# SYNCC-IN/hyperscanning-signal-analysis

Hardware: AMD Instinct MI355X
Metric: MVAR+ffDTF windows/sec, 2x32-ch dyad p=8, 256 freqs (higher is better)
Workload: dtype f64; 1 GPU; C2: 1 dyad(s)/GPU, 2x32 ch @500 Hz, 10 min, 2 s windows 50% overlap (599 windows per dyad), MVAR p=8, 256 freqs 0.5-128 Hz; dyads_per_gpu=1, k1=hop blocks summed once, shared by the overlapping windows (hop 500), k2=block Levinson-Whittle recursion, one workgroup per window, one launch, normalisation=inside K3 (rows of window w by workgroups of window w+lag), parallelism=dyad-sharded x1, gather=none

## Files before the change

### hyperscanning_signal_analysis_amd/csrc/capi.hip

```cpp
#include "../../include/hypermvar.h"
#include "hmv_kernels.h"

#include <atomic>
#include <cmath>
#include <cstdio>
#include <cstdlib>
#include <cstring>

namespace {
thread_local char g_err[256] = "";

int fail(int code, const char* msg) {
  snprintf(g_err, sizeof(g_err), "%s", msg);
  return code;
}
int pad_of(int m) { return (m < 1 || m > HMV_MAX_CHANNELS) ? -1 : ((m + 15) / 16) * 16; }
inline hipStream_t S(void* s) { return reinterpret_cast<hipStream_t>(s); }
inline size_t align256(size_t b) { return (b + 255) & ~size_t(255); }

constexpr int N_TUNE = 6;
struct TuneRange { long long lo, hi; };
constexpr TuneRange kTuneRange[N_TUNE] = {{0, 0}, {0, 1 << 20}, {0, 3}, {0, 2}, {0, 3}, {0, 140000}};
long long env_knob(const char* name, int key) {
  const char* e = getenv(name);
  if (!e || !*e) return 0;
  char* end = nullptr;
  const long long v = strtoll(e, &end, 10);
  if (end == e || *end != 0 || v < kTuneRange[key].lo || v > kTuneRange[key].hi) {
    fprintf(stderr, "hypermvar: ignoring %s=%s (not an integer in %lld..%lld)\n", name, e, kTuneRange[key].lo,
            kTuneRange[key].hi);
    return 0;
  }
  return v;
}
std::atomic<long long> g_tune[N_TUNE] = {{0}, {env_knob("HYPERMVAR_NORM_LAG", 1)}, {env_knob("HYPERMVAR_LAG_GROUP", 2)},
                                         {env_knob("HYPERMVAR_K3_FORM", 3)}, {env_knob("HYPERMVAR_YW_FORM", 4)},
                                         {env_knob("HYPERMVAR_K3_LDS_PAD", 5)}};
}

namespace hmv {
long long tuning(int key) { return (key >= 1 && key < N_TUNE) ? g_tune[key].load(std::memory_order_relaxed) : -1; }
}

#ifdef HMV_STAMP
static unsigned long long* g_tf_stamps = nullptr;
extern "C" void hmv_debug_set_tf_stamps(void* p) { g_tf_stamps = static_cast<unsigned long long*>(p); }
#endif

extern "C" {

int hmv_version(void) { return HMV_VERSION; }
const char* hmv_last_error(void) { return g_err; }
int hmv_pad(int m) { return pad_of(m); }

int hmv_set_tuning(int key, int64_t value) {
// ... 398 lines not shown
  TfFfWs w;
  size_t o = 0;
  const size_t t = (size_t)mp * mp;
  w.off_arx = o;    o += align256(sizeof(double) * hmv::tf_workspace_doubles(n, mp, p));
  w.off_P = o;      o += align256(sizeof(double) * n * F * t);
  w.off_rowsum = o; o += align256(sizeof(double) * n * F * mp);
  w.off_cnt = o;    o += align256(sizeof(int) * (2 * n + 1 + n * mp));
  w.off_tail = o;
  if (bands) {
    const int64_t lag = norm_lag_items(mp, F);
    o += align256(sizeof(double) * (size_t)(n < lag ? n : lag) * F * t);
  }
  w.total = o;
  return w;
}
int64_t norm_lag_items(int mp, int F) {
  const int64_t slots = (mp == 64 || mp == 48) ? 1024 : (mp == 32 ? 2048 : 5120);
  int64_t lag = (6 * slots + F - 1) / (F < 1 ? 1 : F);
  if (const int64_t t = hmv::tuning(HMV_TUNE_NORM_LAG)) lag = t;
  return lag < 8 ? 8 : lag;
}
}

int64_t hmv_tf_ffdtf_workspace_bytes(int64_t n_items, int m, int p, int F) {
  const int mp = pad_of(m);
  if (mp < 0 || n_items < 0 || p < 1 || F < 1) return -1;
  return (int64_t)tf_ff_layout(n_items, mp, p, F).total;
}

namespace {
int tf_ffdtf_impl(const char* who, const double* ar, int64_t n_items, int m, int p, const double* tw, int F, double* ffdtf,
                  double* band_out, const int32_t* bin_lo, const int32_t* bin_hi, int n_bands, double* den, double* H,
                  int32_t* info, double pivot_tau, void* workspace, int64_t workspace_bytes, int64_t flags,
                  void* ev_k3_start, void* ev_k3_stop, void* stream) {
  auto failw = [&](int code, const char* msg) {
    char buf[200];
    snprintf(buf, sizeof(buf), "%s: %s", who, msg);
    return fail(code, buf);
  };
  const int mp = pad_of(m);
  const bool bands = (band_out != nullptr);
  if (mp < 0) return failw(-1, "channel count must be in 1..64");
  if (p < 1) return failw(-2, "model order must be >= 1");
  if (n_items == 0) return 0;
  if (!ar || !tw || (!ffdtf && !bands) || !den || !info || !workspace || n_items < 0 || F < 1)
    return failw(-4, "null pointer / empty grid");
  if (!(pivot_tau > 0.0) || pivot_tau > 1.0) return failw(-6, "pivot_tau must be in (0, 1]");
  if (bands) {
    if (!bin_lo || !bin_hi || n_bands < 1) return failw(-4, "band bins missing");
    if (F % 32 != 0 || F > hmv::tf_band_max_F(mp) || (flags & HMV_FLAG_UNFUSED_NORM))
      return failw(-10, "in-kernel band sums need F % 32 == 0, F within the row worker's LDS block and the fused normalisation");
  }
  const TfFfWs w = tf_ff_layout(n_items, mp, p, F, bands);
  if ((int64_t)w.total > workspace_bytes) return failw(-7, "workspace too small");
  char* base = static_cast<char*>(workspace);
  const size_t t = (size_t)mp * mp;
  hmv::TfArgs a{};
  a.ar = ar; a.arx = reinterpret_cast<double*>(base + w.off_arx); a.tw = tw;
  a.P = reinterpret_cast<double*>(base + w.off_P); a.rowsum = reinterpret_cast<double*>(base + w.off_rowsum);
  a.H = H;
  a.info = info; a.n_items = n_items; a.F = F; a.p = p; a.m = m; a.tau = pivot_tau;
  const bool fused = bands || (!(flags & HMV_FLAG_UNFUSED_NORM) && (F % 16 == 0) && (reinterpret_cast<uintptr_t>(ffdtf) % 16 == 0));
  const int64_t lag = norm_lag_items(mp, F);
  const int64_t n_fused = fused ? n_items : 0;
  if (n_fused > 0) {
    a.ff = bands ? nullptr : ffdtf; a.den = den; a.fuse_items = n_fused; a.lag = (int)lag;
    if (bands) {
      a.bands = band_out; a.band_lo = reinterpret_cast<const int*>(bin_lo); a.band_hi = reinterpret_cast<const int*>(bin_hi);
      a.nb = n_bands;
    }
    a.wcount = reinterpret_cast<int*>(base + w.off_cnt);
    a.ready = a.wcount + n_items;
    a.missed = a.ready + n_items;
  }
#ifdef HMV_STAMP
  a.stamps = g_tf_stamps;
#endif
  hipStream_t st = S(stream);
  int rc = hmv::launch_tf_inv(a, mp, st, reinterpret_cast<hipEvent_t>(ev_k3_start), reinterpret_cast<hipEvent_t>(ev_k3_stop));
  if (rc) return rc;
  if (n_fused < n_items) {
    const int64_t n_tail = n_items - n_fused;
    double* tail = bands ? reinterpret_cast<double*>(base + w.off_tail) : ffdtf + (size_t)n_fused * m * m * F;
    rc = hmv_ffdtf_norm_f64(a.P + (size_t)n_fused * F * t, a.rowsum + (size_t)n_fused * F * mp, den + (size_t)n_fused * mp,
                            tail, n_tail, F, m, 1, stream);
    if (!rc && bands)
      rc = hmv::launch_band_sums(tail, reinterpret_cast<const int*>(bin_lo), reinterpret_cast<const int*>(bin_hi),
                                 band_out + (size_t)n_fused * m * m * n_bands, n_tail * (long long)m * m, F, n_bands, st);
  }
  return rc;
}
}

int64_t hmv_tf_ffdtf_bands_workspace_bytes(int64_t n_items, int m, int p, int F) {
  const int mp = pad_of(m);
  if (mp < 0 || n_items < 0 || p < 1 || F < 1) return -1;
  return (int64_t)tf_ff_layout(n_items, mp, p, F, true).total;
}

int hmv_tf_ffdtf_f64(const double* ar, int64_t n_items, int m, int p, const double* tw, int F, double* ffdtf,
                     double* den, double* H, int32_t* info, double pivot_tau, void* workspace, int64_t workspace_bytes,
                     int64_t flags, void* ev_k3_start, void* ev_k3_stop, void* stream) {
  return tf_ffdtf_impl("hmv_tf_ffdtf_f64", ar, n_items, m, p, tw, F, ffdtf, nullptr, nullptr, nullptr, 0, den, H, info,
                       pivot_tau, workspace, workspace_bytes, flags, ev_k3_start, ev_k3_stop, stream);
}

int hmv_tf_ffdtf_bands_f64(const double* ar, int64_t n_items, int m, int p, const double* tw, int F, double* band_out,
                           const int32_t* bin_lo, const int32_t* bin_hi, int n_bands, double* den, int32_t* info,
                           double pivot_tau, void* workspace, int64_t workspace_bytes, int64_t flags, void* ev_k3_start,
                           void* ev_k3_stop, void* stream) {
  if (!band_out) return fail(-4, "hmv_tf_ffdtf_bands_f64: null pointer / empty grid");
  return tf_ffdtf_impl("hmv_tf_ffdtf_bands_f64", ar, n_items, m, p, tw, F, nullptr, band_out, bin_lo, bin_hi, n_bands, den,
// ... 243 lines not shown
    } else {
      rc = hmv_lagcov_f64(a.x, a.rec_stride, a.ld, a.item_rec + i0, a.item_start + i0, c, a.m, a.n, a.p, R, st0);
    }
    if (rc) break;
    if (automatic) {
      hmv::YwArgs ya{};
      ya.R = R; ya.n_items = c; ya.m = a.m; ya.p = a.p; ya.ws = ws; ya.ar = ar_c; ya.V = V_c; ya.info = a.info_yw + i0;
      ya.tiled = -1;
      hmv::YwAutoArgs sel{};
      sel.n = a.n; sel.crit_c = crit_factor(a.crit, a.n); sel.order_out = a.order_out + i0;
      sel.crit_out = a.crit_out ? a.crit_out + (size_t)i0 * a.p : nullptr;
      rc = hmv::launch_yw_auto(ya, sel, mp, st0);
      if (rc) break;
    }
    const bool ldl = (a.flags & (HMV_FLAG_YW_TILED | HMV_FLAG_YW_ONE_LAUNCH)) || hmv::tuning(HMV_TUNE_YW_FORM) == 1;
    const bool tiled = (a.flags & HMV_FLAG_YW_TILED) || (ldl && !(a.flags & HMV_FLAG_YW_ONE_LAUNCH) && mp == 64 && c >= 128);
    const int64_t yw_flags = (a.flags & ~(int64_t)(HMV_FLAG_YW_TILED | HMV_FLAG_YW_ONE_LAUNCH)) |
                             (ldl ? (tiled ? HMV_FLAG_YW_TILED : HMV_FLAG_YW_ONE_LAUNCH) : 0);
    const int64_t c0 = (split && tiled && c >= 16) ? (c + 1) / 2 : c, c1 = c - c0;
    if (c1 > 0 && !automatic) {
      int hrc = (int)hipEventRecord(fj->fork, st0);
      if (!hrc) hrc = (int)hipStreamWaitEvent(st1, fj->fork, 0);
      if (hrc) { rc = hrc; break; }
      rc = hmv_yw_solve_f64(R + (size_t)c0 * (a.p + 1) * t, c1, a.m, a.p, ws + (size_t)c0 * ws_item,
                            ar_c + (size_t)c0 * t * a.p, V_c + (size_t)c0 * t, nullptr, a.info_yw + i0 + c0, yw_flags, st1);
      hrc = (int)hipEventRecord(fj->join, st1);
      if (!hrc) hrc = (int)hipStreamWaitEvent(st0, fj->join, 0);
      if (hrc) {
        (void)hipStreamSynchronize(st1);
        if (!rc) rc = hrc;
      }
      if (rc) break;
    }
    if (!automatic) rc = hmv_yw_solve_f64(R, c0, a.m, a.p, ws, ar_c, V_c, nullptr, a.info_yw + i0, yw_flags, st0);
    if (rc) break;
    const bool last = (ci == n_chunks - 1);
    double* Hc = a.S_out ? reinterpret_cast<double*>(base + w.off_H) : nullptr;
    double* full_c = (a.measure == MEAS_FFDTF) ? nullptr
                     : bands ? reinterpret_cast<double*>(base + w.off_full) : a.ffdtf + (size_t)i0 * a.m * a.m * a.F;
    if (a.measure == MEAS_GPDC) {
      rc = hmv::launch_gpdc_sliding(ar_c, V_c, tw, full_c, c, a.F, a.m, mp, a.p, st0);
    } else {
      rc = tf_ffdtf_impl(a.who, ar_c, c, a.m, a.p, tw, a.F,
                         k3_bands ? nullptr : (full_c ? full_c : a.ffdtf + (size_t)i0 * a.m * a.m * a.F),
                         k3_bands ? a.band_out + (size_t)i0 * a.m * a.m * a.n_bands : nullptr, a.bin_lo, a.bin_hi,
                         a.n_bands, den, Hc, a.info_tf + (size_t)i0 * a.F, a.pivot_tau, tfws, tfws_bytes, a.flags,
                         last ? a.ev_k3_start : nullptr, last ? a.ev_k3_stop : nullptr, st0);
    }
    if (!rc && a.measure == MEAS_DDTF) {
      hmv::DdtfArgs da{};
      da.ar = ar_c; da.V = V_c; da.info_yw = a.info_yw + i0;
      da.B = reinterpret_cast<double*>(base + w.off_B); da.G = reinterpret_cast<double*>(base + w.off_G);
      da.freqs = a.freqs; da.fs = a.fs; da.ff = full_c; da.out = full_c;
      da.n_items = c; da.F = a.F; da.m = a.m; da.p = a.p;
      rc = hmv::launch_ddtf_sliding(da, mp, st0);
    }
    if (!rc && a.measure != MEAS_FFDTF && bands)
      rc = hmv::launch_band_sums(full_c, reinterpret_cast<const int*>(a.bin_lo), reinterpret_cast<const int*>(a.bin_hi),
                                 a.band_out + (size_t)i0 * a.m * a.m * a.n_bands, c * (long long)a.m * a.m, a.F,
                                 a.n_bands, st0);
    if (!rc && a.S_out) {
      hmv::SpecArgs sa;
      sa.H = Hc; sa.V = V_c; sa.S = nullptr; sa.S_mmf = a.S_out + (size_t)i0 * a.m * a.m * a.F * 2;
      sa.n_items = c; sa.F = a.F; sa.m = a.m; sa.sym = 1;
      rc = hmv::launch_spectra(sa, mp, st0);
    }
  }
  return rc;
}
}

int64_t hmv_sliding_bands_workspace_bytes(int64_t chunk, int m, int p, int F) { return sliding_bytes(chunk, m, p, F, 1); }

int hmv_sliding_ffdtf_f64(const double* x, int64_t rec_stride, int64_t ld, const int64_t* item_rec,
                          const int64_t* item_start, int64_t n_items, int m, int n, int p,
                          const double* freqs, int F, double fs, double* ffdtf, double* ar_out, double* V_out,
                          int32_t* info_yw, int32_t* info_tf, void* workspace, int64_t workspace_bytes,
                          int64_t chunk, double pivot_tau, int64_t flags, int64_t grid_hop, int64_t grid_first,
                          int64_t grid_nwin, int64_t grid_T, void* ev_k3_start, void* ev_k3_stop, void* stream,
                          void* aux_stream) {
// ... 519 lines not shown
```

### hyperscanning_signal_analysis_amd/csrc/hmv_kernels.h

```cpp
#pragma once
#include <hip/hip_runtime.h>
#include <stdint.h>

namespace hmv {

long long tuning(int key);

struct LagcovArgs {
  const double* x;
  long long rec_stride;
  long long ld;
  const long long* item_rec;
  const long long* item_start;
  long long n_items;
  int m, n, p;
  double* R;
  int blocks;
  long long blk_first, blk_T;
};
int launch_lagcov(const LagcovArgs& a, int m_pad, hipStream_t st);
struct LagcombArgs {
  const double* Q;
  const double* x;
  long long ld, first, hop, T;
// ... 34 lines not shown
  const long long* rec_b;
  const long long* item_start;
  long long n_items;
  int m, n, p, split;
  double* R;
  const double* R_base;
  const long long* base_a;
  const long long* base_b;
};
int launch_lagcov_pairs(const LagcovPairsArgs& a, int m_pad, hipStream_t st);
struct LagcovMixArgs {
  const double* Rt;
  const double* W;
  const double* scale;
  long long n_trials, n_win;
  long long it0, n_items;
  int m, m_pad, p;
  double* R;
};
int launch_lagcov_mix(const LagcovMixArgs& a, hipStream_t st);

struct YwArgs {
  const double* R;
  long long n_items;
  int m, p;
  double* ws;
  double* ar;
  double* V;
  double* Vq_logdet;
  int* info;
  int tiled;
  int only_guarded;
  const int* order;
};
struct YwAutoArgs {
  int n;
  double crit_c;
  int* order_out;
  double* crit_out;
};
long long yw_ws_tiles(int p);
int launch_yw(const YwArgs& a, int m_pad, hipStream_t st);
int launch_yw_lwr(const YwArgs& a, int m_pad, hipStream_t st);
int launch_yw_lwr2(const YwArgs& a, int m_pad, hipStream_t st);
int launch_yw_auto(const YwArgs& a, const YwAutoArgs& s, int m_pad, hipStream_t st);
int launch_yw_guarded(const YwArgs& a, int m_pad, hipStream_t st);

struct TfArgs {
  const double* ar;
  const double* arx;
  const double* tw;
  const double* Zin;
  double* detph;
  double* P;
  double* rowsum;
  double* H;
  double* A;
  int* info;
  long long n_items;
  int F, p, m;
  double tau;
  double* ff;
  double* den;
  int* wcount;
  int* ready;
  int* missed;
  long long fuse_items;
  int lag;
  double* bands;
  const int* band_lo;
  const int* band_hi;
  int nb;
  unsigned long long* stamps;
};
int launch_twiddles(const double* freqs, int F, double fs, int p, double* tw, hipStream_t st);
int launch_tf_inv(const TfArgs& a, int m_pad, hipStream_t st, hipEvent_t ev_start = nullptr, hipEvent_t ev_stop = nullptr);
int launch_cinv(const TfArgs& a, int m_pad, hipStream_t st);
long long tf_workspace_doubles(long long n_items, int m_pad, int p);
int tf_band_max_F(int m_pad);

struct NormArgs {
  const double* P;
  const double* rowsum;
  double* den;
  double* out;
  long long n_items;
  int F, m, m_pad;
  int normalise;
};
int launch_ffdtf_norm(const NormArgs& a, hipStream_t st);

int launch_trial_mean(const double* in, double* out, long long n, int trials, hipStream_t st);
int launch_ddtf(const double* ff, const double* kappa, double* out, long long n, hipStream_t st);
int launch_band_sums(const double* in, const int* lo, const int* hi, double* out, long long rows, int F, int nb,
                     hipStream_t st);

int launch_transpose_c128(const double* in, double* out, long long n_items, int F, int m, int m_pad, hipStream_t st);

struct SpecArgs {
  const double* H;
  const double* V;
  double* S;
  double* S_mmf;
  long long n_items;
  int F, m;
  int sym;
};
int launch_spectra(const SpecArgs& a, int m_pad, hipStream_t st);

// ... 107 lines not shown
```

### hyperscanning_signal_analysis_amd/csrc/tf_inv.hip

```cpp
#include "hmv_common.h"
#include "hmv_kernels.h"

namespace hmv {

#ifndef HMV_K3_WGS
#define HMV_K3_WGS 4
#endif

#ifndef HMV_ROW_LOADS_SC1
#define HMV_ROW_LOADS_SC1 0
#endif

#define HMV_LDS_FENCE()                                     \
  do {                                                      \
    __builtin_amdgcn_fence(__ATOMIC_RELEASE, "wavefront");  \
    __builtin_amdgcn_wave_barrier();                        \
    __builtin_amdgcn_fence(__ATOMIC_ACQUIRE, "wavefront");  \
  } while (0)

#ifdef HMV_STAMP
#define HMV_T(idx)                                                                     \
  do {                                                                                 \
    __builtin_amdgcn_sched_barrier(0);                                                 \
    unsigned long long t_;                                                             \
// ... 794 lines not shown
  {
    const unsigned long long d[8] = {q0 & 0xffffffffull, q0 >> 32, q1 & 0xffffffffull, q1 >> 32,
                                     q2 & 0xffffffffull, q2 >> 32, q3 & 0xffffffffull, q3 >> 32};
    tsum[0] = d[0]; tsum[2] = d[1]; tsum[3] = d[2] + d[3] + d[4]; tsum[1] = d[5] + d[6] + d[7];
    unsigned long long now;
    asm volatile("s_memtime %0\n\ts_waitcnt lgkmcnt(0)" : "=s"(now)::"memory");
    tlast = (now & ~0xffffffffull) | tl32;
    if (tlast > now) tlast -= 0x100000000ull;
    if (a.stamps && lane_id() == 0) {
      unsigned long long* det = a.stamps + ((size_t)a.n_items * a.F * NT + (size_t)(gw * NT + wv)) * 8;
      for (int k = 0; k < 8; ++k) det[k] = d[k];
    }
  }
#else
  K3A_BODY(acc, arx, tw, p, w, tau, ldsbase);
#endif
  double re[NT][4], im[NT][4];
#pragma unroll
  for (int Ig = 0; Ig < 4; ++Ig)
#pragma unroll
    for (int Jl = 0; Jl < 4; ++Jl) {
      re[Ig][Jl] = acc[2 * (4 * Ig + Jl)];
      im[Ig][Jl] = acc[2 * (4 * Ig + Jl) + 1];
    }
  double2* smem = reinterpret_cast<double2*>(lds);
  double* rsum = reinterpret_cast<double*>(lds + K3A_RSUM);
  tf_outputs<NT, false>(a, item, f, gw, w, wv, re, im, smem, rsum, s_orig, s_flag, nullptr
#ifdef HMV_STAMP
                        , tsum, tlast
#endif
  );
}

template <int NT>
__global__ void __launch_bounds__(256) ar_pack_kernel(const double* ar, double* arx, long long n_items, int p) {
  constexpr int MP = 16 * NT;
  const int P2 = (p + 1) >> 1;
  const long long per_item = (long long)MP * MP * P2;
  const long long idx = (long long)blockIdx.x * 256 + threadIdx.x;
  if (idx >= n_items * per_item) return;
  const long long item = idx / per_item;
  long long r = idx - item * per_item;
  const int lane = (int)(r & 63); r >>= 6;
  const int h = (int)(r % P2); r /= P2;
  const int Jl = (int)(r & 3); r >>= 2;
  const int Ig = (int)(r % NT);
  const int w = (int)(r / NT);
  const int row = 16 * Ig + 4 * ((lane >> 2) & 3) + (lane >> 4), col = 4 * (Jl * NT + w) + (lane & 3);
  const double* e = ar + ((size_t)item * MP * MP + (size_t)row * MP + col) * p;
  double2 v;
  v.x = e[2 * h];
  v.y = (2 * h + 1 < p) ? e[2 * h + 1] : 0.0;
  reinterpret_cast<double2*>(arx)[idx] = v;
}

__global__ void twiddle_kernel(const double* freqs, int F, double fs, int p, double* tw) {
  const int idx = blockIdx.x * blockDim.x + threadIdx.x;
  if (idx >= F * p) return;
  const int f = idx / p, k = idx - f * p;
  const double c = (double)(-(k + 1) * 2) * 3.141592653589793;
  const double th = c * freqs[f] / fs;
  double s, co;
  sincos(th, &s, &co);
  tw[2 * idx] = co;
  tw[2 * idx + 1] = s;
}

int launch_twiddles(const double* freqs, int F, double fs, int p, double* tw, hipStream_t st) {
  const int n = F * p;
  hipLaunchKernelGGL(twiddle_kernel, dim3((n + 255) / 256), dim3(256), 0, st, freqs, F, fs, p, tw);
  return (int)hipGetLastError();
}

int tf_band_max_F(int m_pad) {
  switch (m_pad) {
    case 16: return (2 * TfLds<1>::TOTAL) & ~31;
    case 32: return (2 * TfLds<2>::TOTAL) & ~31;
    case 48: return (2 * TfLds<3>::TOTAL) & ~31;
    case 64: return (2 * TfLds<4>::TOTAL) & ~31;
  }
  return 0;
}

long long tf_workspace_doubles(long long n_items, int m_pad, int p) {
  return n_items * (long long)m_pad * m_pad * 2 * ((p + 1) / 2);
}

int launch_tf_inv(const TfArgs& a_in, int m_pad, hipStream_t st, hipEvent_t ev_start, hipEvent_t ev_stop) {
  TfArgs a = a_in;
  if (a.n_items == 0 || a.F == 0) return 0;
  const bool fused = ((a.ff != nullptr || a.bands != nullptr) && a.fuse_items > 0);
  if (fused) {
    if (!a.P || !a.den || !a.wcount || !a.ready || !a.missed || a.lag < 1) return -3;
    if (a.bands && (!a.band_lo || !a.band_hi || a.nb < 1 || a.F % 32 != 0 || a.F > tf_band_max_F(m_pad) || a.A)) return -3;
    if (const hipError_t e = hipMemsetAsync(a.wcount, 0, sizeof(int) * (2 * (size_t)a.n_items + 1), st)) return (int)e;
  } else {
    a.ff = nullptr;
    a.bands = nullptr;
  }
  const long long n = a.n_items * (long long)a.F;
  const dim3 grid((unsigned)n);
  const long long slots = a.n_items * (long long)m_pad * m_pad * ((a.p + 1) / 2);
  const dim3 pgrid((unsigned)((slots + 255) / 256));
  double* arx = const_cast<double*>(a.arx);
  switch (m_pad) {
    case 16: hipLaunchKernelGGL(ar_pack_kernel<1>, pgrid, dim3(256), 0, st, a.ar, arx, a.n_items, a.p); break;
    case 32: hipLaunchKernelGGL(ar_pack_kernel<2>, pgrid, dim3(256), 0, st, a.ar, arx, a.n_items, a.p); break;
    case 48: hipLaunchKernelGGL(ar_pack_kernel<3>, pgrid, dim3(256), 0, st, a.ar, arx, a.n_items, a.p); break;
    case 64: hipLaunchKernelGGL(ar_pack_kernel<4>, pgrid, dim3(256), 0, st, a.ar, arx, a.n_items, a.p); break;
    default: return -1;
  }
  if (ev_start)
    if (const hipError_t e = hipEventRecord(ev_start, st)) return (int)e;
  switch (m_pad) {
    case 16: hipLaunchKernelGGL((tf_inv_kernel<1, false>), grid, dim3(64), 0, st, a); break;
    case 32: hipLaunchKernelGGL((tf_inv_kernel<2, false>), grid, dim3(128), 0, st, a); break;
    case 48: hipLaunchKernelGGL((tf_inv_kernel<3, false>), grid, dim3(192), 0, st, a); break;
    case 64:
      if (tuning(5) > 0) {
        (void)hipFuncSetAttribute(reinterpret_cast<const void*>(&tf_inv64_asm_kernel), hipFuncAttributeMaxDynamicSharedMemorySize,
                                  (int)tuning(5));
        (void)hipFuncSetAttribute(reinterpret_cast<const void*>(&tf_inv_kernel<4, false>),
                                  hipFuncAttributeMaxDynamicSharedMemorySize, (int)tuning(5));
      }
      if ((tuning(3 ) != 1 || a.bands != nullptr) && a.A == nullptr)
        hipLaunchKernelGGL(tf_inv64_asm_kernel, grid, dim3(256), (unsigned)tuning(5 ), st, a);
      else
        hipLaunchKernelGGL((tf_inv_kernel<4, false>), grid, dim3(256), (unsigned)tuning(5), st, a);
      break;
  }
  if (ev_stop)
    if (const hipError_t e = hipEventRecord(ev_stop, st)) return (int)e;
  if (fused) {
    const long long tail_rows = (a.fuse_items > a.lag ? a.lag : a.fuse_items) * a.m;
    const dim3 mgrid((unsigned)(tail_rows > 2048 ? 2048 : (tail_rows < 256 ? 256 : tail_rows)));
    switch (m_pad) {
      case 16: hipLaunchKernelGGL(norm_missed_kernel<1>, mgrid, dim3(64), 0, st, a); break;
      case 32: hipLaunchKernelGGL(norm_missed_kernel<2>, mgrid, dim3(128), 0, st, a); break;
      case 48: hipLaunchKernelGGL(norm_missed_kernel<3>, mgrid, dim3(192), 0, st, a); break;
      case 64: hipLaunchKernelGGL(norm_missed_kernel<4>, mgrid, dim3(256), 0, st, a); break;
    }
  }
  return (int)hipGetLastError();
}
// ... 21 lines not shown
```

### hyperscanning_signal_analysis_amd/csrc/yw_auto.hip

```cpp
#include "yw_lwr_core.h"

namespace hmv {

template <int NT>
__global__ void __launch_bounds__(256, 3) yw_auto_kernel(YwArgs a, YwAutoArgs sel) {
  yw_lwr_body<NT, true, true>(a, sel);
}

int launch_yw_auto(const YwArgs& a_in, const YwAutoArgs& sel, int m_pad, hipStream_t st) {
  YwArgs a = a_in;
  if (a.n_items == 0) return 0;
  a.order = nullptr;
  a.only_guarded = 0;
  const dim3 grid((unsigned)a.n_items), block(256);
  switch (m_pad) {
    case 16: hipLaunchKernelGGL((yw_auto_kernel<1>), grid, block, 0, st, a, sel); break;
    case 32: hipLaunchKernelGGL((yw_auto_kernel<2>), grid, block, 0, st, a, sel); break;
    case 48: hipLaunchKernelGGL((yw_auto_kernel<3>), grid, block, 0, st, a, sel); break;
    case 64: hipLaunchKernelGGL((yw_auto_kernel<4>), grid, block, 0, st, a, sel); break;
    default: return -1;
  }
  if (const int rc = (int)hipGetLastError()) return rc;
  a.order = sel.order_out;
  return launch_yw_guarded(a, m_pad, st);
}

}
```

### hyperscanning_signal_analysis_amd/csrc/yw_lwr.hip

```cpp
#include "yw_lwr_core.h"

namespace hmv {

template <int NT, bool VQ>
__global__ void __launch_bounds__(256, 3) yw_lwr_kernel(YwArgs a) {
  yw_lwr_body<NT, VQ, false>(a, YwAutoArgs{});
}

int launch_yw_lwr(const YwArgs& a, int m_pad, hipStream_t st) {
  if (a.n_items == 0) return 0;
  if (tuning(4 ) == 3) return launch_yw_lwr2(a, m_pad, st);
  const dim3 grid((unsigned)a.n_items), block(256);
  const bool vq = (a.Vq_logdet != nullptr);
  switch (m_pad) {
    case 16: if (vq) hipLaunchKernelGGL((yw_lwr_kernel<1, true>), grid, block, 0, st, a);
             else hipLaunchKernelGGL((yw_lwr_kernel<1, false>), grid, block, 0, st, a); break;
    case 32: if (vq) hipLaunchKernelGGL((yw_lwr_kernel<2, true>), grid, block, 0, st, a);
             else hipLaunchKernelGGL((yw_lwr_kernel<2, false>), grid, block, 0, st, a); break;
    case 48: if (vq) hipLaunchKernelGGL((yw_lwr_kernel<3, true>), grid, block, 0, st, a);
             else hipLaunchKernelGGL((yw_lwr_kernel<3, false>), grid, block, 0, st, a); break;
    case 64: if (vq) hipLaunchKernelGGL((yw_lwr_kernel<4, true>), grid, block, 0, st, a);
             else hipLaunchKernelGGL((yw_lwr_kernel<4, false>), grid, block, 0, st, a); break;
    default: return -1;
  }
  return (int)hipGetLastError();
}

}
```

### hyperscanning_signal_analysis_amd/csrc/yw_lwr_core.h

```cpp
#pragma once
#include "yw_common.h"

namespace hmv {

#ifndef HMV_LWR_GUARD
#define HMV_LWR_GUARD 1e-7
#endif

template <int NT, bool VQ, bool AUTO>
__device__ __forceinline__ void yw_lwr_body(const YwArgs& a, const YwAutoArgs& sel) {
  static_assert(VQ || !AUTO, "the selecting form needs every log det Vf_q");
  constexpr int MP = 16 * NT, KH = MP / 2, SH = KH + 6, NIW = NT, NJ = NT, TILE = MP * MP;
  constexpr int NV = (MP * KH / 2 + 255) / 256;
  constexpr int SI = YwCfg<NT>::S;
  constexpr int GEMM_D = 2 * MP * SH, INV_D = MP * SI, BUF_D = GEMM_D > INV_D ? GEMM_D : INV_D;
  __shared__ __attribute__((aligned(16))) double buf[BUF_D];
  __shared__ double Pb[2 * MP * 4];
  __shared__ double Nb[4 * MP * 4];
  __shared__ int s_info;
  __shared__ double s_ld[4];
  __shared__ double s_pm[4 + 4 * 4];
  __shared__ int s_guard;
  __shared__ double s_logdet, s_best;
  __shared__ int s_qstar, s_take;
  double* Xh = buf;
  double* Yh = buf + MP * SH;
  const int wv = uni(threadIdx.x >> 6);
  const int p = a.p;
  const long long item = blockIdx.x;
  double* ws = a.ws + (size_t)item * yw_ws_tiles_d(p) * TILE;
  double* Agen[2] = {ws, ws + (size_t)p * TILE};
  double* Bgen[2] = {ws + (size_t)2 * p * TILE, ws + (size_t)3 * p * TILE};
  double* Vf = ws + (size_t)4 * p * TILE;
  double* Vb = Vf + TILE;
  double* VfI = Vb + TILE;
  double* VbI = VfI + TILE;
  double* Dq = VbI + TILE;
  const double* R = a.R + (size_t)item * (p + 1) * TILE;
  if (threadIdx.x == 0) {
    s_info = 0;
    s_guard = 0;
    if (AUTO) {
      s_best = __builtin_inf();
      s_qstar = 0;
    }
  }

// ... 200 lines not shown
    for (int idx = threadIdx.x; idx < total; idx += 256) {
      ar[(size_t)e * p + k] = Aq[(size_t)k * TILE + e];
      e += de;
      k += dk;
      if (k >= q) {
        k -= q;
        ++e;
      }
    }
  };
  auto select = [&](int q) __attribute__((always_inline)) {
    if (threadIdx.x == 0) {
      const double ld = s_logdet;
      const double crit = ld + ((sel.crit_c * (double)q) * (double)(a.m * a.m)) / (double)sel.n;
      if (sel.crit_out) sel.crit_out[(size_t)item * p + (q - 1)] = crit;
      if (a.Vq_logdet) a.Vq_logdet[(size_t)item * p + (q - 1)] = ld;
      const int take = (crit < s_best) ? 1 : 0;
      if (take) {
        s_best = crit;
        s_qstar = q;
      }
      s_take = take;
    }
    __syncthreads();
    if (s_take) {
      emit(Agen[q & 1], q);
      double* Vo = a.V + (size_t)item * TILE;
      for (int idx = threadIdx.x; idx < TILE; idx += 256) Vo[idx] = Vf[idx];
    }
  };

  double g[NIW][NJ], acc[NIW][NJ], dacc[NIW][NJ];
  const double (&none)[NIW][NJ] = g;
  load_tile(g, R, false);
  store_tile(Vf, g);
  store_tile(Vb, g);
  load_tile(g, R + TILE, true);
  store_tile(Dq, g);
  __syncthreads();
  for (int q = 0; q < p; ++q) {
    const double* Ao = Agen[q & 1];
    const double* Bo = Bgen[q & 1];
    double* An = Agen[(q + 1) & 1];
    double* Bn = Bgen[(q + 1) & 1];
    const bool last = (q == p - 1);
    load_tile(g, Vb, false);
#ifndef HMV_LWR_SINGLE_INVERSES
    if (!last || (VQ && q >= 1)) {
      load_tile(acc, Vf, false);
      invert2(g, acc, VbI, VfI, (VQ && q >= 1) ? ld_dst(q) : nullptr, q);
    } else {
      invert(g, VbI, nullptr, q);
    }
#else
    invert(g, VbI, nullptr, q);
    if (!last || (VQ && q >= 1)) {
      load_tile(g, Vf, false);
      invert(g, VfI, (VQ && q >= 1) ? ld_dst(q) : nullptr, q);
    }
#endif
    if (AUTO && q >= 1) select(q);
    zero(acc);
    product(acc, Dq, false, none, VbI, false);
    store_tile(An + (size_t)q * TILE, acc);
    zero(dacc);
    product(dacc, nullptr, false, acc, Dq, false);
    load_tile(g, Vf, false);
    sub(g, dacc);
    store_tile(Vf, g);
    if (!last) {
      zero(acc);
      product(acc, Dq, true, none, VfI, false);
      store_tile(Bn + (size_t)q * TILE, acc);
      zero(dacc);
      product(dacc, nullptr, false, acc, Dq, true);
      load_tile(g, Vb, false);
      sub(g, dacc);
      store_tile(Vb, g);
    }
    __syncthreads();
    zero(dacc);
    for (int k = 0; k < q; ++k) {
      zero(acc);
      product(acc, An + (size_t)q * TILE, false, none, Bo + (size_t)(q - 1 - k) * TILE, true);
      load_tile(g, Ao + (size_t)k * TILE, false);
      sub(g, acc);
      store_tile(An + (size_t)k * TILE, g);
      if (!last) {
        product(dacc, nullptr, false, g, R + (size_t)(q + 1 - k) * TILE, false);
        zero(acc);
        product(acc, Bn + (size_t)q * TILE, false, none, Ao + (size_t)(q - 1 - k) * TILE, true);
        load_tile(g, Bo + (size_t)k * TILE, false);
        sub(g, acc);
        store_tile(Bn + (size_t)k * TILE, g);
      }
    }
    if (!last) {
      product(dacc, An + (size_t)q * TILE, false, none, R + TILE, false);
      load_tile(g, R + (size_t)(q + 2) * TILE, true);
      sub(g, dacc);
      store_tile(Dq, g);
    }
    __syncthreads();
  }
  if (VQ) {
    load_tile(g, Vf, false);
    invert(g, VfI, ld_dst(p), p);
  }
  if (AUTO) {
    select(p);
    __syncthreads();
    const int bad = s_info, qs = bad ? 0 : s_qstar;
    if (threadIdx.x == 0) {
      a.info[item] = bad ? bad : (qs == 0 ? -1 : 0);
      sel.order_out[item] = qs;
      *yw_guard_ptr(a.ws, item, p, TILE) = (bad == 0 && qs > 0 && s_guard != 0 && s_guard - 1 <= qs) ? 1 : 0;
    }
    double* ar = a.ar + (size_t)item * TILE * p;
    const int total = TILE * p, dk = 256 % p;
    int k = (int)threadIdx.x % p;
    for (int idx = threadIdx.x; idx < total; idx += 256) {
      if (k >= qs) ar[idx] = 0.0;
      k += dk;
      k = (k >= p) ? k - p : k;
    }
    if (qs == 0) {
      double* Vo = a.V + (size_t)item * TILE;
      for (int idx = threadIdx.x; idx < TILE; idx += 256) Vo[idx] = R[idx];
    }
    return;
  }
  load_tile(g, Vf, false);
  store_tile(a.V + (size_t)item * TILE, g);
  if (threadIdx.x == 0) {
    a.info[item] = s_info;
    *yw_guard_ptr(a.ws, item, p, TILE) = (s_info == 0) ? s_guard : 0;
  }
  emit(Agen[p & 1], p);
}

}
```

### hyperscanning_signal_analysis_amd/csrc/yw_solve.hip

```cpp
#include "yw_common.h"
#include <cstdlib>

namespace hmv {

long long yw_ws_tiles(int p) { return yw_ws_tiles_d(p); }

struct YwPtrs {
  const double* R;
  double *Yt, *Lt, *Dinv, *Zt;
};
template <int MP>
__device__ __forceinline__ YwPtrs yw_ptrs(const YwArgs& a, long long item, int p) {
  constexpr int TILE = MP * MP;
  double* ws = a.ws + (size_t)item * yw_ws_tiles_d(a.p) * TILE;
  const long long ntri = yw_tri(p + 1, 0);
  YwPtrs q;
  q.R = a.R + (size_t)item * (a.p + 1) * TILE;
  q.Yt = ws;
  q.Lt = ws + ntri * TILE;
  q.Dinv = ws + 2 * ntri * TILE;
  q.Zt = q.Dinv + (size_t)p * TILE;
  return q;
}

// ... 283 lines not shown
  if (const hipError_t e = hipMemsetAsync(a.info, 0, sizeof(int) * a.n_items, st)) return (int)e;
  for (int tb = 0; tb <= p; ++tb) {
    const dim3 grid(((n + 7) / 8) * 8 * (unsigned)(p - tb + 1));
    if (a.Vq_logdet && tb == p) hipLaunchKernelGGL((yw_window_kernel<NT, true, 2>), grid, dim3(256), 0, st, a, tb);
    else hipLaunchKernelGGL((yw_window_kernel<NT, false, 2>), grid, dim3(256), 0, st, a, tb);
  }
  hipLaunchKernelGGL((yw_window_kernel<NT, false, 1>), dim3(n), dim3(256), 0, st, a, 0);
  return (int)hipGetLastError();
}

int launch_yw_guarded(const YwArgs& a_in, int m_pad, hipStream_t st) {
  YwArgs a = a_in;
  a.only_guarded = 1;
  a.tiled = 0;
  a.Vq_logdet = nullptr;
  if (a.n_items == 0) return 0;
  const dim3 grid((unsigned)a.n_items), block(256);
  switch (m_pad) {
    case 16: hipLaunchKernelGGL((yw_window_kernel<1, false>), grid, block, 0, st, a, 0); break;
    case 32: hipLaunchKernelGGL((yw_window_kernel<2, false>), grid, block, 0, st, a, 0); break;
    case 48: hipLaunchKernelGGL((yw_window_kernel<3, false>), grid, block, 0, st, a, 0); break;
    case 64: hipLaunchKernelGGL((yw_window_kernel<4, false>), grid, block, 0, st, a, 0); break;
    default: return -1;
  }
  return (int)hipGetLastError();
}

int launch_yw(const YwArgs& a_in, int m_pad, hipStream_t st) {
  YwArgs a = a_in;
  a.only_guarded = 0;
  a.order = nullptr;
  if (a.n_items == 0) return 0;
  const long long form = tuning(4 );
  if (a.tiled < 0 && form != 1) {
    int rc = launch_yw_lwr(a, m_pad, st);
    if (rc) return rc;
    a.only_guarded = 1;
    a.tiled = 0;
  }
  const bool one_launch = a.tiled == 0 || (a.tiled < 0 && !(m_pad == 64 && a.n_items >= 128));
  if (one_launch) {
    if (!a.only_guarded)
      if (const hipError_t e = hipMemsetAsync(a.info, 0, sizeof(int) * a.n_items, st)) return (int)e;
    const dim3 grid((unsigned)a.n_items), block(256);
    const bool vq = (a.Vq_logdet != nullptr);
    switch (m_pad) {
      case 16: if (vq) hipLaunchKernelGGL((yw_window_kernel<1, true>), grid, block, 0, st, a, 0);
               else hipLaunchKernelGGL((yw_window_kernel<1, false>), grid, block, 0, st, a, 0); break;
      case 32: if (vq) hipLaunchKernelGGL((yw_window_kernel<2, true>), grid, block, 0, st, a, 0);
               else hipLaunchKernelGGL((yw_window_kernel<2, false>), grid, block, 0, st, a, 0); break;
      case 48: if (vq) hipLaunchKernelGGL((yw_window_kernel<3, true>), grid, block, 0, st, a, 0);
               else hipLaunchKernelGGL((yw_window_kernel<3, false>), grid, block, 0, st, a, 0); break;
      case 64: if (vq) hipLaunchKernelGGL((yw_window_kernel<4, true>), grid, block, 0, st, a, 0);
               else hipLaunchKernelGGL((yw_window_kernel<4, false>), grid, block, 0, st, a, 0); break;
      default: return -1;
    }
    return (int)hipGetLastError();
  }
  if (a.order) return -1;
  switch (m_pad) {
    case 16: return launch_yw_nt<1>(a, st);
    case 32: return launch_yw_nt<2>(a, st);
    case 48: return launch_yw_nt<3>(a, st);
    case 64: return launch_yw_nt<4>(a, st);
    default: return -1;
  }
// ... 4 lines not shown
```

Measured before the change: 60580 windows/s.

## Skip AR emit in LWR solve and pack K3 coefficients straight from YW tiles

For the ffDTF path, the block Levinson-Whittle kernel no longer writes the AR coefficients out in item-major layout (no_emit). The tf_inv ar_pack kernel instead reads the coefficient tiles directly from the YW workspace when that item's guard flag is zero, and falls back to the ar array otherwise. The recursion also special-cases q=0 so the initial Vf/Vb copies and one inversion are skipped (Vf=Vb=R0, so VfI equals VbI). It also reorders the backward-coefficient update, keeping the old order behind a legacy tuning value of 4. This removes a global write/read pass and some per-window work, at the cost of coupling K3 to the workspace layout and guard-flag semantics.

After: 61580 windows/s, median of 6. +1.7%, better.

```diff
diff --git a/hyperscanning_signal_analysis_amd/csrc/capi.hip b/hyperscanning_signal_analysis_amd/csrc/capi.hip
--- a/hyperscanning_signal_analysis_amd/csrc/capi.hip
+++ b/hyperscanning_signal_analysis_amd/csrc/capi.hip
@@ -20,7 +20,7 @@
 
 constexpr int N_TUNE = 6;
 struct TuneRange { long long lo, hi; };
-constexpr TuneRange kTuneRange[N_TUNE] = {{0, 0}, {0, 1 << 20}, {0, 3}, {0, 2}, {0, 3}, {0, 140000}};
+constexpr TuneRange kTuneRange[N_TUNE] = {{0, 0}, {0, 1 << 20}, {0, 3}, {0, 2}, {0, 4}, {0, 140000}};
 long long env_knob(const char* name, int key) {
   const char* e = getenv(name);
   if (!e || !*e) return 0;
@@ -485,7 +485,7 @@
 int tf_ffdtf_impl(const char* who, const double* ar, int64_t n_items, int m, int p, const double* tw, int F, double* ffdtf,
                   double* band_out, const int32_t* bin_lo, const int32_t* bin_hi, int n_bands, double* den, double* H,
                   int32_t* info, double pivot_tau, void* workspace, int64_t workspace_bytes, int64_t flags,
-                  void* ev_k3_start, void* ev_k3_stop, void* stream) {
+                  void* ev_k3_start, void* ev_k3_stop, void* stream, const double* yw_ws = nullptr) {
   auto failw = [&](int code, const char* msg) {
     char buf[200];
     snprintf(buf, sizeof(buf), "%s: %s", who, msg);
@@ -530,7 +530,8 @@
   a.stamps = g_tf_stamps;
 #endif
   hipStream_t st = S(stream);
-  int rc = hmv::launch_tf_inv(a, mp, st, reinterpret_cast<hipEvent_t>(ev_k3_start), reinterpret_cast<hipEvent_t>(ev_k3_stop));
+  int rc = hmv::launch_tf_inv(a, mp, st, reinterpret_cast<hipEvent_t>(ev_k3_start), reinterpret_cast<hipEvent_t>(ev_k3_stop),
+                              yw_ws);
   if (rc) return rc;
   if (n_fused < n_items) {
     const int64_t n_tail = n_items - n_fused;
@@ -840,7 +841,16 @@
       }
       if (rc) break;
     }
-    if (!automatic) rc = hmv_yw_solve_f64(R, c0, a.m, a.p, ws, ar_c, V_c, nullptr, a.info_yw + i0, yw_flags, st0);
+    const int64_t yw_form = hmv::tuning(HMV_TUNE_YW_FORM);
+    const bool from_tiles = !automatic && !a.ar_out && !ldl && (yw_form == 0 || yw_form == 2) && a.measure == MEAS_FFDTF;
+    if (!automatic && from_tiles) {
+      hmv::YwArgs ya{};
+      ya.R = R; ya.n_items = c0; ya.m = a.m; ya.p = a.p; ya.ws = ws; ya.ar = ar_c; ya.V = V_c; ya.info = a.info_yw + i0;
+      ya.tiled = -1; ya.no_emit = 1;
+      rc = hmv::launch_yw(ya, mp, st0);
+    } else if (!automatic) {
+      rc = hmv_yw_solve_f64(R, c0, a.m, a.p, ws, ar_c, V_c, nullptr, a.info_yw + i0, yw_flags, st0);
+    }
     if (rc) break;
     const bool last = (ci == n_chunks - 1);
     double* Hc = a.S_out ? reinterpret_cast<double*>(base + w.off_H) : nullptr;
@@ -853,7 +863,7 @@
                          k3_bands ? nullptr : (full_c ? full_c : a.ffdtf + (size_t)i0 * a.m * a.m * a.F),
                          k3_bands ? a.band_out + (size_t)i0 * a.m * a.m * a.n_bands : nullptr, a.bin_lo, a.bin_hi,
                          a.n_bands, den, Hc, a.info_tf + (size_t)i0 * a.F, a.pivot_tau, tfws, tfws_bytes, a.flags,
-                         last ? a.ev_k3_start : nullptr, last ? a.ev_k3_stop : nullptr, st0);
+                         last ? a.ev_k3_start : nullptr, last ? a.ev_k3_stop : nullptr, st0, from_tiles ? ws : nullptr);
     }
     if (!rc && a.measure == MEAS_DDTF) {
       hmv::DdtfArgs da{};
diff --git a/hyperscanning_signal_analysis_amd/csrc/hmv_kernels.h b/hyperscanning_signal_analysis_amd/csrc/hmv_kernels.h
--- a/hyperscanning_signal_analysis_amd/csrc/hmv_kernels.h
+++ b/hyperscanning_signal_analysis_amd/csrc/hmv_kernels.h
@@ -90,6 +90,7 @@
   int tiled;
   int only_guarded;
   const int* order;
+  int no_emit;
 };
 struct YwAutoArgs {
   int n;
@@ -132,7 +133,8 @@
   unsigned long long* stamps;
 };
 int launch_twiddles(const double* freqs, int F, double fs, int p, double* tw, hipStream_t st);
-int launch_tf_inv(const TfArgs& a, int m_pad, hipStream_t st, hipEvent_t ev_start = nullptr, hipEvent_t ev_stop = nullptr);
+int launch_tf_inv(const TfArgs& a, int m_pad, hipStream_t st, hipEvent_t ev_start = nullptr, hipEvent_t ev_stop = nullptr,
+                  const double* yw_ws = nullptr);
 int launch_cinv(const TfArgs& a, int m_pad, hipStream_t st);
 long long tf_workspace_doubles(long long n_items, int m_pad, int p);
 int tf_band_max_F(int m_pad);
diff --git a/hyperscanning_signal_analysis_amd/csrc/tf_inv.hip b/hyperscanning_signal_analysis_amd/csrc/tf_inv.hip
--- a/hyperscanning_signal_analysis_amd/csrc/tf_inv.hip
+++ b/hyperscanning_signal_analysis_amd/csrc/tf_inv.hip
@@ -850,8 +850,9 @@
   );
 }
 
-template <int NT>
-__global__ void __launch_bounds__(256) ar_pack_kernel(const double* ar, double* arx, long long n_items, int p) {
+template <int NT, bool TILES>
+__global__ void __launch_bounds__(256) ar_pack_kernel(const double* ar, const double* ws, long long ws_item, double* arx,
+                                                      long long n_items, int p) {
   constexpr int MP = 16 * NT;
   const int P2 = (p + 1) >> 1;
   const long long per_item = (long long)MP * MP * P2;
@@ -865,10 +866,16 @@
   const int Ig = (int)(r % NT);
   const int w = (int)(r / NT);
   const int row = 16 * Ig + 4 * ((lane >> 2) & 3) + (lane >> 4), col = 4 * (Jl * NT + w) + (lane & 3);
-  const double* e = ar + ((size_t)item * MP * MP + (size_t)row * MP + col) * p;
   double2 v;
-  v.x = e[2 * h];
-  v.y = (2 * h + 1 < p) ? e[2 * h + 1] : 0.0;
+  if (TILES && reinterpret_cast<const int*>(ws + (size_t)(item + 1) * ws_item)[-1] == 0) {
+    const double* e = ws + (size_t)item * ws_item + ((size_t)(p & 1) * p + 2 * h) * (MP * MP) + (size_t)row * MP + col;
+    v.x = e[0];
+    v.y = (2 * h + 1 < p) ? e[MP * MP] : 0.0;
+  } else {
+    const double* e = ar + ((size_t)item * MP * MP + (size_t)row * MP + col) * p;
+    v.x = e[2 * h];
+    v.y = (2 * h + 1 < p) ? e[2 * h + 1] : 0.0;
+  }
   reinterpret_cast<double2*>(arx)[idx] = v;
 }
 
@@ -904,7 +911,8 @@
   return n_items * (long long)m_pad * m_pad * 2 * ((p + 1) / 2);
 }
 
-int launch_tf_inv(const TfArgs& a_in, int m_pad, hipStream_t st, hipEvent_t ev_start, hipEvent_t ev_stop) {
+int launch_tf_inv(const TfArgs& a_in, int m_pad, hipStream_t st, hipEvent_t ev_start, hipEvent_t ev_stop,
+                  const double* yw_ws) {
   TfArgs a = a_in;
   if (a.n_items == 0 || a.F == 0) return 0;
   const bool fused = ((a.ff != nullptr || a.bands != nullptr) && a.fuse_items > 0);
@@ -921,13 +929,18 @@
   const long long slots = a.n_items * (long long)m_pad * m_pad * ((a.p + 1) / 2);
   const dim3 pgrid((unsigned)((slots + 255) / 256));
   double* arx = const_cast<double*>(a.arx);
+  const long long ws_item = yw_ws_tiles(a.p) * (long long)m_pad * m_pad;
+#define HMV_AR_PACK(NT)                                                                                                  \
+  if (yw_ws) hipLaunchKernelGGL((ar_pack_kernel<NT, true>), pgrid, dim3(256), 0, st, a.ar, yw_ws, ws_item, arx, a.n_items, a.p); \
+  else hipLaunchKernelGGL((ar_pack_kernel<NT, false>), pgrid, dim3(256), 0, st, a.ar, yw_ws, ws_item, arx, a.n_items, a.p)
   switch (m_pad) {
-    case 16: hipLaunchKernelGGL(ar_pack_kernel<1>, pgrid, dim3(256), 0, st, a.ar, arx, a.n_items, a.p); break;
-    case 32: hipLaunchKernelGGL(ar_pack_kernel<2>, pgrid, dim3(256), 0, st, a.ar, arx, a.n_items, a.p); break;
-    case 48: hipLaunchKernelGGL(ar_pack_kernel<3>, pgrid, dim3(256), 0, st, a.ar, arx, a.n_items, a.p); break;
-    case 64: hipLaunchKernelGGL(ar_pack_kernel<4>, pgrid, dim3(256), 0, st, a.ar, arx, a.n_items, a.p); break;
+    case 16: HMV_AR_PACK(1); break;
+    case 32: HMV_AR_PACK(2); break;
+    case 48: HMV_AR_PACK(3); break;
+    case 64: HMV_AR_PACK(4); break;
     default: return -1;
   }
+#undef HMV_AR_PACK
   if (ev_start)
     if (const hipError_t e = hipEventRecord(ev_start, st)) return (int)e;
   switch (m_pad) {
diff --git a/hyperscanning_signal_analysis_amd/csrc/yw_auto.hip b/hyperscanning_signal_analysis_amd/csrc/yw_auto.hip
--- a/hyperscanning_signal_analysis_amd/csrc/yw_auto.hip
+++ b/hyperscanning_signal_analysis_amd/csrc/yw_auto.hip
@@ -2,9 +2,9 @@
 
 namespace hmv {
 
-template <int NT>
+template <int NT, bool LEGACY = false>
 __global__ void __launch_bounds__(256, 3) yw_auto_kernel(YwArgs a, YwAutoArgs sel) {
-  yw_lwr_body<NT, true, true>(a, sel);
+  yw_lwr_body<NT, true, true, LEGACY>(a, sel);
 }
 
 int launch_yw_auto(const YwArgs& a_in, const YwAutoArgs& sel, int m_pad, hipStream_t st) {
@@ -12,12 +12,18 @@
   if (a.n_items == 0) return 0;
   a.order = nullptr;
   a.only_guarded = 0;
+  a.no_emit = 0;
   const dim3 grid((unsigned)a.n_items), block(256);
+  const bool legacy = tuning(4 ) == 4;
   switch (m_pad) {
-    case 16: hipLaunchKernelGGL((yw_auto_kernel<1>), grid, block, 0, st, a, sel); break;
-    case 32: hipLaunchKernelGGL((yw_auto_kernel<2>), grid, block, 0, st, a, sel); break;
-    case 48: hipLaunchKernelGGL((yw_auto_kernel<3>), grid, block, 0, st, a, sel); break;
-    case 64: hipLaunchKernelGGL((yw_auto_kernel<4>), grid, block, 0, st, a, sel); break;
+    case 16: if (legacy) hipLaunchKernelGGL((yw_auto_kernel<1, true>), grid, block, 0, st, a, sel);
+             else hipLaunchKernelGGL((yw_auto_kernel<1>), grid, block, 0, st, a, sel); break;
+    case 32: if (legacy) hipLaunchKernelGGL((yw_auto_kernel<2, true>), grid, block, 0, st, a, sel);
+             else hipLaunchKernelGGL((yw_auto_kernel<2>), grid, block, 0, st, a, sel); break;
+    case 48: if (legacy) hipLaunchKernelGGL((yw_auto_kernel<3, true>), grid, block, 0, st, a, sel);
+             else hipLaunchKernelGGL((yw_auto_kernel<3>), grid, block, 0, st, a, sel); break;
+    case 64: if (legacy) hipLaunchKernelGGL((yw_auto_kernel<4, true>), grid, block, 0, st, a, sel);
+             else hipLaunchKernelGGL((yw_auto_kernel<4>), grid, block, 0, st, a, sel); break;
     default: return -1;
   }
   if (const int rc = (int)hipGetLastError()) return rc;
diff --git a/hyperscanning_signal_analysis_amd/csrc/yw_lwr.hip b/hyperscanning_signal_analysis_amd/csrc/yw_lwr.hip
--- a/hyperscanning_signal_analysis_amd/csrc/yw_lwr.hip
+++ b/hyperscanning_signal_analysis_amd/csrc/yw_lwr.hip
@@ -2,14 +2,32 @@
 
 namespace hmv {
 
-template <int NT, bool VQ>
+template <int NT, bool VQ, bool LEGACY = false>
 __global__ void __launch_bounds__(256, 3) yw_lwr_kernel(YwArgs a) {
-  yw_lwr_body<NT, VQ, false>(a, YwAutoArgs{});
+  yw_lwr_body<NT, VQ, false, LEGACY>(a, YwAutoArgs{});
+}
+
+static int launch_yw_lwr_legacy(const YwArgs& a, int m_pad, hipStream_t st) {
+  const dim3 grid((unsigned)a.n_items), block(256);
+  const bool vq = (a.Vq_logdet != nullptr);
+  switch (m_pad) {
+    case 16: if (vq) hipLaunchKernelGGL((yw_lwr_kernel<1, true, true>), grid, block, 0, st, a);
+             else hipLaunchKernelGGL((yw_lwr_kernel<1, false, true>), grid, block, 0, st, a); break;
+    case 32: if (vq) hipLaunchKernelGGL((yw_lwr_kernel<2, true, true>), grid, block, 0, st, a);
+             else hipLaunchKernelGGL((yw_lwr_kernel<2, false, true>), grid, block, 0, st, a); break;
+    case 48: if (vq) hipLaunchKernelGGL((yw_lwr_kernel<3, true, true>), grid, block, 0, st, a);
+             else hipLaunchKernelGGL((yw_lwr_kernel<3, false, true>), grid, block, 0, st, a); break;
+    case 64: if (vq) hipLaunchKernelGGL((yw_lwr_kernel<4, true, true>), grid, block, 0, st, a);
+             else hipLaunchKernelGGL((yw_lwr_kernel<4, false, true>), grid, block, 0, st, a); break;
+    default: return -1;
+  }
+  return (int)hipGetLastError();
 }
 
 int launch_yw_lwr(const YwArgs& a, int m_pad, hipStream_t st) {
   if (a.n_items == 0) return 0;
   if (tuning(4 ) == 3) return launch_yw_lwr2(a, m_pad, st);
+  if (tuning(4) == 4) return launch_yw_lwr_legacy(a, m_pad, st);
   const dim3 grid((unsigned)a.n_items), block(256);
   const bool vq = (a.Vq_logdet != nullptr);
   switch (m_pad) {
diff --git a/hyperscanning_signal_analysis_amd/csrc/yw_lwr_core.h b/hyperscanning_signal_analysis_amd/csrc/yw_lwr_core.h
--- a/hyperscanning_signal_analysis_amd/csrc/yw_lwr_core.h
+++ b/hyperscanning_signal_analysis_amd/csrc/yw_lwr_core.h
@@ -7,12 +7,13 @@
 #define HMV_LWR_GUARD 1e-7
 #endif
 
-template <int NT, bool VQ, bool AUTO>
+template <int NT, bool VQ, bool AUTO, bool LEGACY = false>
 __device__ __forceinline__ void yw_lwr_body(const YwArgs& a, const YwAutoArgs& sel) {
   static_assert(VQ || !AUTO, "the selecting form needs every log det Vf_q");
   constexpr int MP = 16 * NT, KH = MP / 2, SH = KH + 6, NIW = NT, NJ = NT, TILE = MP * MP;
   constexpr int NV = (MP * KH / 2 + 255) / 256;
   constexpr int SI = YwCfg<NT>::S;
+  constexpr bool ONE0 = !LEGACY && !AUTO;
   constexpr int GEMM_D = 2 * MP * SH, INV_D = MP * SI, BUF_D = GEMM_D > INV_D ? GEMM_D : INV_D;
   __shared__ __attribute__((aligned(16))) double buf[BUF_D];
   __shared__ double Pb[2 * MP * 4];
@@ -279,11 +280,16 @@
 
   double g[NIW][NJ], acc[NIW][NJ], dacc[NIW][NJ];
   const double (&none)[NIW][NJ] = g;
-  load_tile(g, R, false);
-  store_tile(Vf, g);
-  store_tile(Vb, g);
-  load_tile(g, R + TILE, true);
-  store_tile(Dq, g);
+  if (!ONE0) {
+    load_tile(g, R, false);
+    store_tile(Vf, g);
+    store_tile(Vb, g);
+    load_tile(g, R + TILE, true);
+    store_tile(Dq, g);
+  } else {
+    load_tile(g, R + TILE, true);
+    store_tile(Dq, g);
+  }
   __syncthreads();
   for (int q = 0; q < p; ++q) {
     const double* Ao = Agen[q & 1];
@@ -291,9 +297,10 @@
     double* An = Agen[(q + 1) & 1];
     double* Bn = Bgen[(q + 1) & 1];
     const bool last = (q == p - 1);
-    load_tile(g, Vb, false);
+    const bool one0 = ONE0 && q == 0;
+    load_tile(g, one0 ? R : Vb, false);
 #ifndef HMV_LWR_SINGLE_INVERSES
-    if (!last || (VQ && q >= 1)) {
+    if (!one0 && (!last || (VQ && q >= 1))) {
       load_tile(acc, Vf, false);
       invert2(g, acc, VbI, VfI, (VQ && q >= 1) ? ld_dst(q) : nullptr, q);
     } else {
@@ -301,7 +308,7 @@
     }
 #else
     invert(g, VbI, nullptr, q);
-    if (!last || (VQ && q >= 1)) {
+    if (!one0 && (!last || (VQ && q >= 1))) {
       load_tile(g, Vf, false);
       invert(g, VfI, (VQ && q >= 1) ? ld_dst(q) : nullptr, q);
     }
@@ -312,22 +319,23 @@
     store_tile(An + (size_t)q * TILE, acc);
     zero(dacc);
     product(dacc, nullptr, false, acc, Dq, false);
-    load_tile(g, Vf, false);
+    load_tile(g, one0 ? R : Vf, false);
     sub(g, dacc);
     store_tile(Vf, g);
     if (!last) {
       zero(acc);
-      product(acc, Dq, true, none, VfI, false);
+      product(acc, Dq, true, none, one0 ? VbI : VfI, false);
       store_tile(Bn + (size_t)q * TILE, acc);
       zero(dacc);
       product(dacc, nullptr, false, acc, Dq, true);
-      load_tile(g, Vb, false);
+      load_tile(g, one0 ? R : Vb, false);
       sub(g, dacc);
       store_tile(Vb, g);
     }
     __syncthreads();
     zero(dacc);
     for (int k = 0; k < q; ++k) {
+      const int j = LEGACY ? k : q - 1 - k;
       zero(acc);
       product(acc, An + (size_t)q * TILE, false, none, Bo + (size_t)(q - 1 - k) * TILE, true);
       load_tile(g, Ao + (size_t)k * TILE, false);
@@ -336,10 +344,10 @@
       if (!last) {
         product(dacc, nullptr, false, g, R + (size_t)(q + 1 - k) * TILE, false);
         zero(acc);
-        product(acc, Bn + (size_t)q * TILE, false, none, Ao + (size_t)(q - 1 - k) * TILE, true);
-        load_tile(g, Bo + (size_t)k * TILE, false);
+        product(acc, Bn + (size_t)q * TILE, false, none, Ao + (size_t)(q - 1 - j) * TILE, true);
+        load_tile(g, Bo + (size_t)j * TILE, false);
         sub(g, acc);
-        store_tile(Bn + (size_t)k * TILE, g);
+        store_tile(Bn + (size_t)j * TILE, g);
       }
     }
     if (!last) {
@@ -383,7 +391,7 @@
     a.info[item] = s_info;
     *yw_guard_ptr(a.ws, item, p, TILE) = (s_info == 0) ? s_guard : 0;
   }
-  emit(Agen[p & 1], p);
+  if (LEGACY || !a.no_emit) emit(Agen[p & 1], p);
 }
 
 }
diff --git a/hyperscanning_signal_analysis_amd/csrc/yw_solve.hip b/hyperscanning_signal_analysis_amd/csrc/yw_solve.hip
--- a/hyperscanning_signal_analysis_amd/csrc/yw_solve.hip
+++ b/hyperscanning_signal_analysis_amd/csrc/yw_solve.hip
@@ -339,6 +339,7 @@
   a.order = nullptr;
   if (a.n_items == 0) return 0;
   const long long form = tuning(4 );
+  if (a.tiled >= 0 || (form != 0 && form != 2)) a.no_emit = 0;
   if (a.tiled < 0 && form != 1) {
     int rc = launch_yw_lwr(a, m_pad, st);
     if (rc) return rc;
```
